# USCbiostats/fmcmc

Hardware: AMD Instinct MI355X
Metric: MH samples/sec (chains x iters / s), 1024 chains, 5-param linreg n=10k (higher is better)
Workload: dtype f64

## Files before the change

### fmcmc_amd/csrc/mh_spec.hpp

```cpp
#pragma once

namespace {

constexpr int SPEC_NT = 768;
constexpr int SPEC_NCW = 8;

__device__ __forceinline__ unsigned lds_ld_u32(const unsigned* p) {
  unsigned v;
  asm volatile("ds_read_b32 %0, %1\n\ts_waitcnt lgkmcnt(0)" : "=v"(v) : "v"((unsigned)(size_t)p) : "memory");
  return v;
}

__device__ __forceinline__ void lds_st_u32(unsigned* p, unsigned v) {
  asm volatile("ds_write_b32 %0, %1" : : "v"((unsigned)(size_t)p), "v"(v) : "memory");
}

__device__ __forceinline__ double lds_ld_f64(const double* p) {
  double v;
  asm volatile("ds_read_b64 %0, %1\n\ts_waitcnt lgkmcnt(0)" : "=v"(v) : "v"((unsigned)(size_t)p) : "memory");
  return v;
}



constexpr int SPEC_ALD = PIPE_KMAX + 1;
constexpr int SPEC_ADS = 7 * PIPE_KMAX + 2 * PIPE_KMAX * SPEC_ALD;

template <int KIND, class SYNC>
__device__ __forceinline__ void spec_owner_adaptive(const SweepArgs& A, int myc, int cl, double* s_th1, const double* s_par,
                                                    SYNC& sync, double* ad) {
  const int lane = threadIdx.x & 63;
  const int k = A.k, kz = A.kz, nsteps = (int)A.nsteps, burnin = (int)A.burnin, thin = (int)A.thin;
  constexpr int LD = SPEC_ALD;
  double* th0 = ad;
  double* th1 = th0 + PIPE_KMAX;
  double* vz = th1 + PIPE_KMAX;
  double* vv = vz + PIPE_KMAX;
  double* vmp = vv + PIPE_KMAX;
  double* vmt = vmp + PIPE_KMAX;
  double* vrs = vmt + PIPE_KMAX;
  double* SigA = vrs + PIPE_KMAX;
  double* SigB = SigA + PIPE_KMAX * LD;
  __shared__ int s_which[4][PIPE_KMAX];
  int kf = 0;
  for (int j = 0; j < k; j++)
    if (!A.fixed[j]) { if (lane == 0) s_which[myc][kf] = j; kf++; }
  const int* which = s_which[myc];
  const double* s_mu = s_par, *s_lb = s_par + 2 * PIPE_KMAX, *s_ub = s_par + 3 * PIPE_KMAX;
  double f0 = 0.0;
  long long abs_iter = 0;
  int nacc = 0, status = A.win_cont ? A.status[cl] : FMCMC_CHAIN_OK, thin_ctr = A.thin_ctr0, have_mean = 0, nerr = 0;
  const int ioff = (int)A.step_off;
  unsigned int bitword = 0;
  double* const Scur = SigA;
  if (lane < k) { double t = A.theta0[(long long)cl * k + lane]; th0[lane] = t; th1[lane] = t; }
  for (int e = lane; e < kf * LD; e += 64) {
    const int a = e / LD, b = e % LD;
    SigA[e] = A.fresh ? ((a == b) ? 1.0 * A.eps : 0.0) : ((b < kf && (b <= a || KIND == FMCMC_KERNEL_ADAPT)) ? A.Sigma[((long long)cl * kf + a) * kf + b] : 0.0);
    SigB[e] = 0.0;
  }
  if (!A.fresh) {
    abs_iter = A.abs_iter[cl];
    if (A.nerrors) nerr = A.nerrors[cl];
    if (KIND == FMCMC_KERNEL_ADAPT) {
      have_mean = A.have_mean[cl];
      if (lane < kf) vmp[lane] = A.mean_prev[(long long)cl * kf + lane];
    }
  }
  wave_sync_lds();
  const int jl = (lane < k) ? lane : 0;
  char* const s_base = reinterpret_cast<char*>(A.samples) + ((long long)cl * k) * A.ldS * 8;
  char* const d_base = A.draws ? reinterpret_cast<char*>(A.draws) + ((long long)cl * k) * A.ldS * 8 : nullptr;
  char* const l_base = A.logpost ? reinterpret_cast<char*>(A.logpost) + (long long)cl * A.ldS * 8 : nullptr;
  const unsigned int lane_off = (unsigned int)((long long)jl * A.ldS * 8);
  unsigned int srow8 = 0;
  const char* const z_base = reinterpret_cast<const char*>(A.fed_z) + ((long long)cl * nsteps) * kz * 8;
  const unsigned int z_lane = (unsigned int)((lane < kz ? lane : 0)) * 8u;
  const double* const lu_row = A.fed_logu + (long long)cl * nsteps;
  auto ld_z = [&](int row) -> double {
    return *reinterpret_cast<const double*>(z_base + (z_lane + (unsigned int)row * (unsigned int)(kz * 8)));
  };
  double z_nx = (lane < kz && nsteps >= 2) ? ld_z(1) : 0.0;
  double lu_nx = (nsteps >= 2) ? lu_row[1] : 0.0;
  bool ram_gate = false;
  auto flush_bits = [&](int i) {
    if (A.accept_bits && lane == 0) {
      unsigned int* w = A.accept_bits + ((long long)cl * A.bits_stride + ((i - 1) >> 5));
      *w = (A.win_cont && i <= 32) ? (*w | bitword) : bitword;
    }
    bitword = 0;
  };

  for (int v = 1; v <= nsteps; v++) {
    const double tot = sync.total(v, []() {});
    const double f1 = finish_logpost(A, th1, tot);
    bool keep_row = false, st_row = false;
    double st_th0 = 0.0, st_dr = 0.0;
    if (v == 1) {
      f0 = f1;
      if (lane < kf) vrs[lane] = (A.win_cont && A.win_sum) ? A.win_sum[(long long)cl * kf + lane] : th0[which[lane]];
      keep_row = true;
    } else if (status == FMCMC_CHAIN_OK) {
      const int i = v;
      if (KIND == FMCMC_KERNEL_RAM) {
        if (ram_gate) {
          double a_n = fmh_exp(f1 - f0);
          if (fmh_isnan(a_n)) a_n = 0.0;
          else if (a_n > 1.0) a_n = 1.0;
          double eta = (double)kf * fmh_exp(A.ram_neg_exp * fmh_log((double)(i + ioff)));
          if (eta > 1.0) eta = 1.0;
          const double zl = (lane < kf) ? vz[lane] : 0.0;
          const double Pj1 = lane_scan_row16(zl * zl);
          const double Pj = dpp_d<0x111>(Pj1);
          const double nrm2 = readlane_d(Pj1, kf - 1);
          double cp = (eta * (a_n - A.arate)) / nrm2;
          if (cp != 0.0 && fmh_isfinite(cp)) {
            double dl, kl;
            const bool okl = ram_coef(cp, Pj, Pj1, zl, dl, kl);
            if (__any(lane < kf && !okl)) {
              nerr += 1;
            } else {
              double* row = Scur + ((lane < kf) ? lane : 0) * LD;
              const double* grow = SigB + ((lane < kf) ? lane : 0) * LD;
              for (int j = 0; j < kf; j++) {
                const double dj = readlane_d(dl, j), kj = readlane_d(kl, j);
                const double sij = row[j];
                const double nw = fmh_fma(grow[j], kj, sij * dj);
                if (lane >= j && lane < kf) row[j] = nw;
              }
              wave_sync_lds();
            }
          }
        }
        abs_iter += 1;
      }
      if (fmh_isnan(f1)) status = FMCMC_CHAIN_NAN_LOGPOST;
      const double ratio = f1 - f0;
      if (status == FMCMC_CHAIN_OK && fmh_isnan(ratio)) status = FMCMC_CHAIN_NAN_RATIO;
      if (status != FMCMC_CHAIN_OK) {
        if (lane == 0) { A.status[cl] = status; A.status_step[cl] = i + ioff; }
        if (lane < k) A.status_theta[(long long)cl * k + lane] = th1[lane];
        flush_bits(i);
      } else {
        const double lu = lu_nx;
        lu_nx = lu_row[v < nsteps ? v : nsteps - 1];
        keep_row = true;
        if (i > burnin) {
          thin_ctr += 1;
        }
        const bool acc = lu < ratio;
        const double dr = (lane < k) ? th1[lane] : 0.0;
        if (acc) {
          if (lane < k) th0[lane] = dr;
          f0 = f1;
          nacc += 1;
          bitword |= (1u << ((i - 1) & 31));
        }
        wave_sync_lds();
        if (i > burnin && thin_ctr == thin) {
          thin_ctr = 0;
          st_row = true;
          st_th0 = (lane < k) ? th0[lane] : 0.0;
          st_dr = dr;
        }
        if (KIND == FMCMC_KERNEL_ADAPT && lane < kf) vrs[lane] = vrs[lane] + th0[which[lane]];
        if (((i - 1) & 31) == 31 || i == nsteps) flush_bits(i);
      }
    }
    if (v == 1 && keep_row && 1 > burnin) {
      thin_ctr += 1;
      if (thin_ctr == thin) {
        thin_ctr = 0;
        if (lane < k) {
          *reinterpret_cast<double*>(s_base + (lane_off + srow8)) = th0[lane];
          if (d_base) *reinterpret_cast<double*>(d_base + (lane_off + srow8)) = th1[lane];
        }
        if (l_base && lane == 0) *reinterpret_cast<double*>(l_base + srow8) = f1;
        srow8 += 8;
      }
    }
    if (v < nsteps) {
      if (status == FMCMC_CHAIN_OK) {
        const int i = v + 1;
        wave_sync_lds();
        if (lane < kz) vz[lane] = z_nx;
        z_nx = (lane < kz) ? ld_z(v + 1 < nsteps ? v + 1 : nsteps - 1) : 0.0;
        wave_sync_lds();
        if (KIND == FMCMC_KERNEL_ADAPT) {
          if (A.until > (double)abs_iter && abs_iter > A.warmup && i + ioff > 2) {
            const double t = (double)(abs_iter - 1);
            double x = 0, mp = 0, mt = 0;
            if (lane < kf) {
              x = th0[which[lane]];
              mp = have_mean ? vmp[lane] : (vrs[lane] / (double)(i + ioff - 1));
              mt = (mp * t + x) / (t + 1);
              vv[lane] = x; vmp[lane] = mp; vmt[lane] = mt;
            }
            wave_sync_lds();
            if (lane < kf) {
              const double c1 = (t - 1) / t, c2 = 1.0 / t;
              int b = 0;
              for (; b + 4 <= kf; b += 4) {
                double pb[4], tb[4], xb[4], sb[4];
#pragma unroll
                for (int u = 0; u < 4; u++) { pb[u] = vmp[b + u]; tb[u] = vmt[b + u]; xb[u] = vv[b + u]; sb[u] = SigA[lane * LD + b + u]; }
#pragma unroll
                for (int u = 0; u < 4; u++) {
                  const double ik = (b + u == lane) ? 1.0 * A.eps : 0.0;
                  const double inner = t * (mp * pb[u]) - (t + 1) * (mt * tb[u]) + x * xb[u] + 1e-5 * ik;
                  SigA[lane * LD + b + u] = c1 * sb[u] + c2 * inner;
                }
              }
              for (; b < kf; b++) {
                double ik = (b == lane) ? 1.0 * A.eps : 0.0;
                double inner = t * (mp * vmp[b]) - (t + 1) * (mt * vmt[b]) + x * vv[b] + 1e-5 * ik;
                SigA[lane * LD + b] = c1 * SigA[lane * LD + b] + c2 * inner;
              }
            }
            wave_sync_lds();
            if (lane < kf) vmp[lane] = mt;
            have_mean = 1;
          }
          abs_iter += 1;
          bool notpd = false;
          for (int j = 0; j < kf; j++) {
            double sacc = 0.0;
            if (lane >= j && lane < kf) {
              sacc = SigA[lane * LD + j];
              int b = 0;
              for (; b + 4 <= j; b += 4) {
                double lb4[4], wb4[4];
#pragma unroll
                for (int u = 0; u < 4; u++) { lb4[u] = SigB[lane * LD + b + u]; wb4[u] = SigB[(b + u) * LD + j]; }
#pragma unroll
                for (int u = 0; u < 4; u++) sacc = fmh_fma(-lb4[u], wb4[u], sacc);
              }
              for (; b < j; b++) sacc = fmh_fma(-SigB[lane * LD + b], SigB[b * LD + j], sacc);
            }
            const double d = readlane_d(sacc, j);
            if (!(d > 0.0) || !fmh_isfinite(d)) { notpd = true; break; }
            if (lane == j) { SigB[j * LD + j] = 1.0; vv[j] = d; }
            else if (lane > j && lane < kf) { SigB[lane * LD + j] = sacc / d; SigB[j * LD + lane] = sacc; }
            wave_sync_lds();
          }
          if (notpd) {
            status = FMCMC_CHAIN_NOT_PD;
            if (lane == 0) { A.status[cl] = status; A.status_step[cl] = i + ioff; }
            if (lane < k) A.status_theta[(long long)cl * k + lane] = th1[lane];
            if (((v - 1) & 31) != 31) flush_bits(v);
          } else {
            if (lane < k) th1[lane] = th0[lane];
            if (lane < kf) vz[lane] = fmh_sqrt(vv[lane]) * vz[lane];
            wave_sync_lds();
            if (lane < kf) {
              double sacc = 0.0;
              for (int b = 0; b < kf; b += 4) {
                double lb4[4], zb4[4];
#pragma unroll
                for (int u = 0; u < 4; u++) { const int bb = (b + u < kf) ? b + u : kf - 1; lb4[u] = SigB[lane * LD + bb]; zb4[u] = vz[bb]; }
#pragma unroll
                for (int u = 0; u < 4; u++) { const double nx = fmh_fma(lb4[u], zb4[u], sacc); sacc = (b + u <= lane) ? nx : sacc; }
              }
              const int j = which[lane];
              th1[j] = reflect1(th0[j] + (s_mu[j] + sacc), s_lb[j], s_ub[j]);
            }
          }
        } else {
          if (lane < kf) {
            double sacc = 0.0;
            for (int b = lane; b >= 0; b--) {
              SigB[lane * LD + b] = sacc;
              sacc = fmh_fma(Scur[lane * LD + b], vz[b], sacc);
            }
            const int j = which[lane];
            th1[j] = th0[j] + sacc;
          }
          ram_gate = (A.until > (double)abs_iter && abs_iter > A.warmup && ((v + 1 + ioff) % A.freq) == 0);
        }
        wave_sync_lds();
        if (lane < k) s_th1[myc * PIPE_KMAX + lane] = th1[lane];
      }
      sync.publish(v + 1);
    } else {
      sync.final();
    }
    if (st_row) {
      if (lane < k) {
        *reinterpret_cast<double*>(s_base + (lane_off + srow8)) = st_th0;
        if (d_base) *reinterpret_cast<double*>(d_base + (lane_off + srow8)) = st_dr;
      }
      if (l_base && lane == 0) *reinterpret_cast<double*>(l_base + srow8) = f1;
      srow8 += 8;
    }
  }
  wave_sync_lds();
  if (lane < k) A.theta0[(long long)cl * k + lane] = th0[lane];
  if (lane == 0) {
    A.f0[cl] = f0;
    A.accept_count[cl] = nacc;
    if (status == FMCMC_CHAIN_OK) { A.status[cl] = FMCMC_CHAIN_OK; A.status_step[cl] = 0; }
    A.abs_iter[cl] = abs_iter;
    if (A.nerrors) A.nerrors[cl] = nerr;
    if (KIND == FMCMC_KERNEL_ADAPT) A.have_mean[cl] = have_mean;
  }
  if (KIND == FMCMC_KERNEL_ADAPT && A.win_sum && lane < kf) A.win_sum[(long long)cl * kf + lane] = vrs[lane];
  const double* Sfin = (KIND == FMCMC_KERNEL_RAM) ? Scur : SigA;
  for (int e = lane; e < kf * kf; e += 64) {
    const int a = e / kf, b = e % kf;
    A.Sigma[((long long)cl * kf + a) * kf + b] = Sfin[a * LD + b];
  }
  if (KIND == FMCMC_KERNEL_ADAPT && lane < kf) A.mean_prev[(long long)cl * kf + lane] = vmp[lane];
}

constexpr int SPEC_KA = 8;

struct SpecSync {
  static constexpr bool PREP_EARLY = false;
  unsigned* s_ready; unsigned* s_done; const double* s_tr; int myc;
  template <class F> __device__ __forceinline__ double total(int v, F&&) const {
    const int lane = threadIdx.x & 63;
    while (lds_ld_u32(&s_done[myc]) < 8u * (unsigned)v) __builtin_amdgcn_s_sleep(1);
    const double* src = s_tr + myc * (8 * PIPE_TRS) + lane;
    const double v0 = src[0 * PIPE_TRS], v1 = src[1 * PIPE_TRS], v2 = src[2 * PIPE_TRS], v3 = src[3 * PIPE_TRS];
    const double v4 = src[4 * PIPE_TRS], v5 = src[5 * PIPE_TRS], v6 = src[6 * PIPE_TRS], v7 = src[7 * PIPE_TRS];
    return wave_xor_sum(((v0 + v1) + (v2 + v3)) + ((v4 + v5) + (v6 + v7)));
  }
  __device__ __forceinline__ void publish(int vn) const {
    asm volatile("s_waitcnt lgkmcnt(0)" ::: "memory");
    if ((threadIdx.x & 63) == 0) __hip_atomic_store(&s_ready[myc], (unsigned)vn, __ATOMIC_RELAXED, __HIP_MEMORY_SCOPE_WORKGROUP);
  }
  __device__ __forceinline__ void final() const {}
};
constexpr unsigned SPEC_FINAL = 0xFFFFFFFFu;
struct SpecSyncB {
  static constexpr bool PREP_EARLY = false;
  unsigned* s_ready; unsigned* s_done; const double* s_tr; int myc;
  mutable unsigned nreq = 1u;
  __device__ __forceinline__ double served() const {
    const int lane = threadIdx.x & 63;
    while (lds_ld_u32(&s_done[myc]) < 8u * nreq) __builtin_amdgcn_s_sleep(1);
    const double* src = s_tr + myc * (8 * PIPE_TRS) + lane;
    const double v0 = src[0 * PIPE_TRS], v1 = src[1 * PIPE_TRS], v2 = src[2 * PIPE_TRS], v3 = src[3 * PIPE_TRS];
    const double v4 = src[4 * PIPE_TRS], v5 = src[5 * PIPE_TRS], v6 = src[6 * PIPE_TRS], v7 = src[7 * PIPE_TRS];
    return wave_xor_sum(((v0 + v1) + (v2 + v3)) + ((v4 + v5) + (v6 + v7)));
  }
  __device__ __forceinline__ void ask() const {
    nreq += 1u;
    asm volatile("s_waitcnt lgkmcnt(0)" ::: "memory");
    if ((threadIdx.x & 63) == 0) __hip_atomic_store(&s_ready[myc], nreq, __ATOMIC_RELAXED, __HIP_MEMORY_SCOPE_WORKGROUP);
  }
  template <class F> __device__ __forceinline__ double total(int, F&&) const { return served(); }
  template <class W> __device__ __forceinline__ bool second(bool need, W&& republish, double& tot2) const {
    if (!need) return false;
    republish();
    ask();
    tot2 = served();
    return true;
  }
  __device__ __forceinline__ void second_idle() const {}
  __device__ __forceinline__ void publish(int) const { ask(); }
  __device__ __forceinline__ void final() const {
    if ((threadIdx.x & 63) == 0) __hip_atomic_store(&s_ready[myc], SPEC_FINAL, __ATOMIC_RELAXED, __HIP_MEMORY_SCOPE_WORKGROUP);
  }
};
constexpr int SPEC_FREQMAX = 8;
template <int KIND, int KX, class SYNC, bool BND = false, int FAM = FMCMC_FAM_GAUSSIAN_LINREG, bool RING = false>
__device__ __forceinline__ void spec_owner_adaptive_reg(const SweepArgs& A, int myc, int cl, double* s_th1, SYNC& sync,
                                                        double* ring = nullptr ) {
  static_assert(!BND || KIND == FMCMC_KERNEL_RAM, "BND is the bounded kernel_ram");
  constexpr bool LG = FAM == FMCMC_FAM_LOGISTIC;
  constexpr int KA = KX > 0 ? KX : SPEC_KA;
  const int lane = threadIdx.x & 63;
  const int k = KX > 0 ? KX : A.k, kz = KX > 0 ? KX : A.kz, kf = (KX > 0 || LG) ? k : kz;
  const int nsteps = (int)A.nsteps, burnin = (int)A.burnin, thin = (int)A.thin;
  const bool rl = lane < k;
  const int jl = rl ? lane : 0;
  const bool fl = lane < kf;
  int pj = jl, sig_lane = k - 1;
  if constexpr (KX == 0 && !LG) {
    int nfree = 0, nfix = 0, mine = 0;
    for (int j = 0; j < k; j++) {
      const bool fx = A.fixed[j] != 0;
      const int pos = fx ? (kf + nfix) : nfree;
      if (pos == lane) mine = j;
      if (j == k - 1) sig_lane = pos;
      nfree += fx ? 0 : 1; nfix += fx ? 1 : 0;
    }
    pj = rl ? mine : 0;
  }
  const double mu_l = A.mu[pj], lb_l = A.lb[pj], ub_l = A.ub[pj];
  double Srow[KA], Lrow[KA];
  double Wrow[KIND == FMCMC_KERNEL_ADAPT ? KA : 1];
  double (&Grow)[KA] = Lrow;
#pragma unroll
  for (int b = 0; b < (KIND == FMCMC_KERNEL_ADAPT ? KA : 1); b++) Wrow[b] = 0.0;
#pragma unroll
  for (int b = 0; b < KA; b++) {
    Lrow[b] = 0.0;
    Srow[b] = (fl && b < kf) ? (A.fresh ? ((b == lane) ? 1.0 * A.eps : 0.0)
                                        : ((b <= lane || KIND == FMCMC_KERNEL_ADAPT) ? A.Sigma[((long long)cl * kf + lane) * kf + b] : 0.0)) : 0.0;
  }
  double th0 = rl ? A.theta0[(long long)cl * k + pj] : 0.0, th1 = th0;
  double f0 = 0.0, mean_prev = 0.0, run_sum = 0.0, zcur = 0.0;
  double Dl = 0.0;
  long long abs_iter = 0;
  int nacc = 0, status = A.win_cont ? A.status[cl] : FMCMC_CHAIN_OK, thin_ctr = A.thin_ctr0, have_mean = 0, nerr = 0;
  const int ioff = (int)A.step_off;
  unsigned int bitword = 0;
  if (!A.fresh) {
    abs_iter = A.abs_iter[cl];
    if (A.nerrors) nerr = A.nerrors[cl];
    if (KIND == FMCMC_KERNEL_ADAPT) {
      have_mean = A.have_mean[cl];
      if (fl) mean_prev = A.mean_prev[(long long)cl * kf + lane];
    }
  }
  char* const s_base = reinterpret_cast<char*>(A.samples) + ((long long)cl * k) * A.ldS * 8;
  char* const d_base = A.draws ? reinterpret_cast<char*>(A.draws) + ((long long)cl * k) * A.ldS * 8 : nullptr;
  char* const l_base = A.logpost ? reinterpret_cast<char*>(A.logpost) + (long long)cl * A.ldS * 8 : nullptr;
  const unsigned int lane_off = (unsigned int)((long long)pj * A.ldS * 8);
  unsigned int srow8 = 0;
  const char* const z_base = reinterpret_cast<const char*>(A.fed_z) + ((long long)cl * nsteps) * kz * 8;
  const unsigned int z_lane = (unsigned int)(fl ? lane : 0) * 8u;
  const double* const lu_row = A.fed_logu + (long long)cl * nsteps;
  const double dn = uniform_d((double)A.n);
  auto ld_z = [&](int row) -> double {
    return *reinterpret_cast<const double*>(z_base + (z_lane + (unsigned int)row * (unsigned int)(kz * 8)));
  };
  double z_nx = (fl && nsteps >= 2) ? ld_z(1) : 0.0;
  double lu_nx = (nsteps >= 2) ? lu_row[1] : 0.0;
  bool ram_gate = false;
  auto flush_bits = [&](int i) {
    if (A.accept_bits && lane == 0) {
      unsigned int* w = A.accept_bits + ((long long)cl * A.bits_stride + ((i - 1) >> 5));
      *w = (A.win_cont && i <= 32) ? (*w | bitword) : bitword;
    }
    bitword = 0;
  };
  auto logpost_of = [&](double tot, double sigma) -> double {
    double f;
    if (sigma < 0.0 || fmh_isnan(sigma)) f = fmh_nan();
    else if (sigma == 0.0) f = -fmh_inf();
    else {
      double t1 = fmh_log(sigma) + FMH_K(FMH_LN_SQRT_2PI);
      double q = (0.5 * tot) / (sigma * sigma);
      f = -(dn * t1) - q;
    }
    if (A.guard && !fmh_isfinite(f)) f = -fmh_inf();
    return f;
  };

  double pre_nt1 = 0.0, pre_ss = 1.0, pre_rs = 1.0, pre_eta = 0.0, pre_Pj = 0.0, pre_Pj1 = 0.0, pre_nrm2 = 1.0;
  double pre_c1 = 0.0, pre_c2 = 0.0;
  double pre_lin = 0.0, pre_pri = 0.0;
  const int nbl = A.intercept + A.p;
  const double hs_l = (LG && lane < nbl && A.lg_hs) ? A.lg_hs[lane] : 0.0;
  bool pre_ok = false;
  auto prepare = [&](int i) {
    if (KIND == FMCMC_KERNEL_ADAPT) {
      const double t = uniform_d((double)(abs_iter - 1));
      pre_c1 = (t - 1) / t;
      pre_c2 = 1.0 / t;
    }
    if constexpr (LG) {
      double lin = 0.0, ss = 0.0;
      for (int j = 0; j < nbl; j++) {
        const double bj = readlane_d(th1, j);
        lin = fmh_fma(bj, readlane_d(hs_l, j), lin);
        ss = fmh_fma(bj, bj, ss);
      }
      pre_lin = lin;
      pre_pri = (A.prior_div != 0.0) ? ss / A.prior_div : 0.0;
      if (KIND == FMCMC_KERNEL_RAM && i >= 2) {
        double eta = (double)kf * fmh_exp(A.ram_neg_exp * fmh_log((double)(i + ioff)));
        if (eta > 1.0) eta = 1.0;
        pre_eta = eta;
        pre_Pj1 = lane_scan_row16(zcur * zcur);
        pre_Pj = dpp_d<0x111>(pre_Pj1);
        pre_nrm2 = readlane_d(pre_Pj1, kf - 1);
      }
      return;
    }
    const double sigma = readlane_d(th1, sig_lane);
    const unsigned sg_hi = (unsigned)(fmh_d2u(sigma) >> 32);
    const bool sg_fast = (sg_hi - 0x00100000u) < 0x7fe00000u;
    const double sg = sg_fast ? sigma : 1.0;
    pre_nt1 = dn * (fmh_log(sg) + FMH_K(FMH_LN_SQRT_2PI));
    pre_ss = sg * sg;
    pre_ok = sg_fast && mfr_div_safe(pre_ss);
    pre_rs = div_recip(pre_ok ? pre_ss : 1.0);
    if (KIND == FMCMC_KERNEL_RAM && i >= 2) {
      double eta = (double)kf * fmh_exp(A.ram_neg_exp * fmh_log((double)(i + ioff)));
      if (eta > 1.0) eta = 1.0;
      pre_eta = eta;
      pre_Pj1 = lane_scan_row16(zcur * zcur);
      pre_Pj = dpp_d<0x111>(pre_Pj1);
      pre_nrm2 = readlane_d(pre_Pj1, kf - 1);
    }
  };
  if (!SYNC::PREP_EARLY) prepare(1);
#ifdef SPEC_STAMP
  unsigned long long stt[8] = {0, 0, 0, 0, 0, 0, 0, 0}, stp = clk();
#define SPEC_ST(i) do { const unsigned long long t_ = clk(); stt[i] += t_ - stp; stp = t_; } while (0)
#else
#define SPEC_ST(i) do { } while (0)
#endif

  for (int v = 1; v <= nsteps; v++) {
    const double tot = sync.total(v, [&]() { prepare(v); });
    SPEC_ST(0);
    const double h = 0.5 * tot;
    double f1;
    if constexpr (LG) {
      f1 = pre_lin - tot;
      if (A.prior_div != 0.0) f1 = f1 - pre_pri;
      if (A.guard && !fmh_isfinite(f1)) f1 = -fmh_inf();
    } else if (pre_ok && mfr_div_safe(h)) f1 = -pre_nt1 - div_finish(h, pre_ss, pre_rs);
    else f1 = logpost_of(tot, readlane_d(th1, sig_lane));
    bool st_row = false;
    double st_th0 = 0.0;
    double st_dr = th1;
    SPEC_ST(1);
    if (v == 1) {
      f0 = f1;
      run_sum = (A.win_cont && A.win_sum && fl) ? A.win_sum[(long long)cl * kf + lane] : th0;
      if (1 > burnin) { thin_ctr += 1; if (thin_ctr == thin) { thin_ctr = 0; st_row = true; st_th0 = th0; } }
      if constexpr (BND) sync.second_idle();
    } else if (status != FMCMC_CHAIN_OK) {
      if constexpr (BND) sync.second_idle();
    } else {
      const int i = v;
      if (KIND == FMCMC_KERNEL_RAM) {
        if (ram_gate) {
          double a_n = fmh_exp(f1 - f0);
          if (fmh_isnan(a_n)) a_n = 0.0;
          else if (a_n > 1.0) a_n = 1.0;
          const double eta = pre_eta, Pj1 = pre_Pj1, Pj = pre_Pj, nrm2 = pre_nrm2;
          const double cp = (eta * (a_n - A.arate)) / nrm2;
          if (cp != 0.0 && fmh_isfinite(cp)) {
            double dl, kl;
            const bool okl = ram_coef(cp, Pj, Pj1, zcur, dl, kl);
            if (__any(fl && !okl)) {
              nerr += 1;
            } else {
              static_for<KA>([&](auto j_) {
                constexpr int j = decltype(j_)::value;
                if (j < kf) {
                  const double dj = row_bcast<j>(dl), kj = row_bcast<j>(kl);
                  Srow[j] = fmh_fma(Grow[j], kj, Srow[j] * dj);
                }
              });
            }
          }
        }
        abs_iter += 1;
        if constexpr (BND) {
          const double th1r = fl ? reflect1(th1, lb_l, ub_l) : th1;
          const bool moved = __any(fl && !(th1r == th1));
          th1 = th1r;
          st_dr = th1r;
          double tot2 = 0.0;
          const bool again = sync.second(moved, [&]() { if (rl) s_th1[myc * PIPE_KMAX + pj] = th1; }, tot2);
          if (again && moved) {
            if constexpr (LG) {
              double lin = 0.0, ss = 0.0;
              for (int j = 0; j < nbl; j++) {
                const double bj = readlane_d(th1, j);
                lin = fmh_fma(bj, readlane_d(hs_l, j), lin);
                ss = fmh_fma(bj, bj, ss);
              }
              f1 = lin - tot2;
              if (A.prior_div != 0.0) f1 = f1 - ss / A.prior_div;
              if (A.guard && !fmh_isfinite(f1)) f1 = -fmh_inf();
            } else {
              f1 = logpost_of(tot2, readlane_d(th1, sig_lane));
            }
          }
        }
      }
      if (fmh_isnan(f1)) status = FMCMC_CHAIN_NAN_LOGPOST;
      const double ratio = f1 - f0;
      if (status == FMCMC_CHAIN_OK && fmh_isnan(ratio)) status = FMCMC_CHAIN_NAN_RATIO;
      if (status != FMCMC_CHAIN_OK) {
        if (lane == 0) { A.status[cl] = status; A.status_step[cl] = i + ioff; }
        if (rl) A.status_theta[(long long)cl * k + pj] = th1;
        flush_bits(i);
      } else {
        const double lu = lu_nx;
        lu_nx = lu_row[v < nsteps ? v : nsteps - 1];
        if (lu < ratio) {
          th0 = th1;
          f0 = f1;
          nacc += 1;
          bitword |= (1u << ((i - 1) & 31));
        }
        if (i > burnin) { thin_ctr += 1; if (thin_ctr == thin) { thin_ctr = 0; st_row = true; st_th0 = th0; } }
        if (KIND == FMCMC_KERNEL_ADAPT) run_sum = run_sum + th0;
        if (((i - 1) & 31) == 31 || i == nsteps) flush_bits(i);
      }
    }
    SPEC_ST(2);
    const int afreq = (KIND == FMCMC_KERNEL_ADAPT && RING) ? A.freq : 1;
    if (KIND == FMCMC_KERNEL_ADAPT && afreq > 1 && ring && fl) ring[(v & (SPEC_FREQMAX - 1)) * PIPE_KMAX + lane] = th0;
    if (v < nsteps) {
      if (status == FMCMC_CHAIN_OK) {
        const int i = v + 1;
        zcur = z_nx;
        z_nx = fl ? ld_z(v + 1 < nsteps ? v + 1 : nsteps - 1) : 0.0;
        bool sig_dirty = (afreq == 1) || v == 1;
        if (KIND == FMCMC_KERNEL_ADAPT) {
          if (A.until > (double)abs_iter && abs_iter > A.warmup && i + ioff > 2 && (afreq == 1 || ((i + ioff) % afreq) == 0)) {
            if (afreq > 1 && i - afreq < 1) {
              status = FMCMC_CHAIN_BAD_WINDOW;
            } else {
              for (int jr = 0; jr < afreq; jr++) {
                const double t = (double)(abs_iter - afreq + jr);
                const double x = (afreq == 1) ? th0 : (fl ? ring[((i - afreq + jr) & (SPEC_FREQMAX - 1)) * PIPE_KMAX + lane] : 0.0);
                const double mp = have_mean ? mean_prev : (run_sum / (double)(i + ioff - 1));
                const double mt = (mp * t + x) / (t + 1);
                const double c1 = (afreq == 1) ? pre_c1 : (t - 1) / t, c2 = (afreq == 1) ? pre_c2 : 1.0 / t;
                static_for<KA>([&](auto b_) {
                  constexpr int b = decltype(b_)::value;
                  if (b < kf) {
                    const double mpb = row_bcast<b>(mp), mtb = row_bcast<b>(mt), xb = row_bcast<b>(x);
                    const double ik = (b == lane) ? 1.0 * A.eps : 0.0;
                    const double inner = t * (mp * mpb) - (t + 1) * (mt * mtb) + x * xb + 1e-5 * ik;
                    Srow[b] = c1 * Srow[b] + c2 * inner;
                  }
                });
                mean_prev = mt;
                have_mean = 1;
              }
              sig_dirty = true;
            }
          }
          abs_iter += 1;
          SPEC_ST(3);
          bool notpd = false;
          if (!RING || (status == FMCMC_CHAIN_OK && sig_dirty)) {
          Dl = 0.0;
          static_for<KA>([&](auto j_) {
            constexpr int j = decltype(j_)::value;
            if (j < kf && (KX > 0 || !notpd)) {
              double sacc = Srow[j];
              static_for<j>([&](auto b_) {
                constexpr int b = decltype(b_)::value;
                sacc = fmac_row_bcast<j, true>(sacc, Wrow[KIND == FMCMC_KERNEL_ADAPT ? b : 0], Lrow[b]);
              });
              const double d = readlane_d(sacc, j);
              const bool badp = !(d > 0.0) || !fmh_isfinite(d);
              if (KX > 0) notpd = notpd || badp;
              if (KX <= 0 && badp) {
                notpd = true;
              } else {
                const double qj = sacc / d;
                Lrow[j] = (lane == j) ? 1.0 : ((lane > j) ? qj : Lrow[j]);
                Wrow[KIND == FMCMC_KERNEL_ADAPT ? j : 0] = sacc;
                Dl = (lane == j) ? d : Dl;
              }
            }
          });
          }
          SPEC_ST(4);
          if (notpd || (RING && status != FMCMC_CHAIN_OK)) {
            if (notpd) status = FMCMC_CHAIN_NOT_PD;
            if (lane == 0) { A.status[cl] = status; A.status_step[cl] = i + ioff; }
            if (rl) A.status_theta[(long long)cl * k + pj] = th1;
            if (((v - 1) & 31) != 31) flush_bits(v);
          } else {
            const double ul = fmh_sqrt(Dl) * zcur;
            double sacc = 0.0;
            static_for<KA>([&](auto b_) {
              constexpr int b = decltype(b_)::value;
              if (b < kf) sacc = fmac_row_bcast<b>(sacc, ul, Lrow[b]);
            });
            th1 = (KX != 0 || LG || fl) ? reflect1(th0 + (mu_l + sacc), lb_l, ub_l) : th0;
          }
        } else {
          double sacc = 0.0;
          static_for<KA>([&](auto r_) {
            constexpr int b = KA - 1 - decltype(r_)::value;
            if (b < kf) { Grow[b] = sacc; sacc = fmac_row_bcast<b>(sacc, zcur, Srow[b]); }
          });
          th1 = (KX != 0 || LG || fl) ? th0 + sacc : th0;
          ram_gate = (A.until > (double)abs_iter && abs_iter > A.warmup && ((v + 1 + ioff) % A.freq) == 0);
        }
        if (rl) s_th1[myc * PIPE_KMAX + pj] = th1;
      }
      sync.publish(v + 1);
    } else {
      sync.final();
    }
    SPEC_ST(5);
    if (st_row) {
      if (rl) {
        *reinterpret_cast<double*>(s_base + (lane_off + srow8)) = st_th0;
        if (d_base) *reinterpret_cast<double*>(d_base + (lane_off + srow8)) = st_dr;
      }
      if (l_base && lane == 0) *reinterpret_cast<double*>(l_base + srow8) = f1;
      srow8 += 8;
    }
    SPEC_ST(6);
    if (!SYNC::PREP_EARLY && v < nsteps) prepare(v + 1);
    SPEC_ST(7);
  }
#ifdef SPEC_STAMP
  __builtin_amdgcn_s_waitcnt(0);
  if (lane < 16 && A.draws) A.draws[(long long)cl * 16 + lane] = (lane < 8) ? (double)stt[lane & 7] : (double)nsteps;
#endif
#undef SPEC_ST
  if (rl) A.theta0[(long long)cl * k + pj] = th0;
  if (lane == 0) {
    A.f0[cl] = f0;
    A.accept_count[cl] = nacc;
    if (status == FMCMC_CHAIN_OK) { A.status[cl] = FMCMC_CHAIN_OK; A.status_step[cl] = 0; }
    A.abs_iter[cl] = abs_iter;
    if (A.nerrors) A.nerrors[cl] = nerr;
    if (KIND == FMCMC_KERNEL_ADAPT) A.have_mean[cl] = have_mean;
  }
#pragma unroll
  for (int b = 0; b < KA; b++)
    if (fl && b < kf) A.Sigma[((long long)cl * kf + lane) * kf + b] = (b <= lane || KIND == FMCMC_KERNEL_ADAPT) ? Srow[b] : 0.0;
  if (KIND == FMCMC_KERNEL_ADAPT && fl) A.mean_prev[(long long)cl * kf + lane] = mean_prev;
  if (KIND == FMCMC_KERNEL_ADAPT && A.win_sum && fl) A.win_sum[(long long)cl * kf + lane] = run_sum;
}

template <int KIND, class SYNC>
__device__ __forceinline__ void mfma_owner_mirror(const SweepArgs& A, int myc, int cl, double* s_th1, SYNC& sync) {
  const int lane = threadIdx.x & 63;
  const int k = A.k, kz = A.kz;
  const int nsteps = (int)A.nsteps, burnin = (int)A.burnin, thin = (int)A.thin;
  const bool rl = lane < k;
  const int jl = rl ? lane : 0;
  const double lb_l = A.lb[jl], ub_l = A.ub[jl];
  double th0 = rl ? A.theta0[(long long)cl * k + lane] : 0.0, th1 = th0;
  double mmu = rl ? (A.fresh ? A.mu[jl] : A.mirror_mu[(long long)cl * k + jl]) : 0.0;
  double msc = rl ? (A.fresh ? A.scale[jl] : A.mirror_scale[(long long)cl * k + jl]) : 0.0;
  double f0 = 0.0, obs_arate = fmh_nan(), th_prev = 0.0;
  long long abs_iter = 0, nzero = 0;
  if (!A.fresh) { abs_iter = A.abs_iter[cl]; obs_arate = A.obs_arate[(long long)cl * k + jl]; }
  int nacc = 0, status = FMCMC_CHAIN_OK, thin_ctr = 0;
  unsigned int bitword = 0;
  char* const s_base = reinterpret_cast<char*>(A.samples) + ((long long)cl * k) * A.ldS * 8;
  char* const d_base = A.draws ? reinterpret_cast<char*>(A.draws) + ((long long)cl * k) * A.ldS * 8 : nullptr;
  char* const l_base = A.logpost ? reinterpret_cast<char*>(A.logpost) + (long long)cl * A.ldS * 8 : nullptr;
  const unsigned int lane_off = (unsigned int)((long long)jl * A.ldS * 8);
  unsigned int srow8 = 0;
  const char* const z_base = reinterpret_cast<const char*>(A.fed_z) + ((long long)cl * nsteps) * kz * 8;
  const unsigned int z_lane = (unsigned int)(jl) * 8u;
  const double* const lu_row = A.fed_logu + (long long)cl * nsteps;
  const double dn = uniform_d((double)A.n);
  auto ld_z = [&](int row) -> double { return *reinterpret_cast<const double*>(z_base + (z_lane + (unsigned int)row * (unsigned int)(kz * 8))); };
  double z_nx = (rl && nsteps >= 2) ? ld_z(1) : 0.0;
  double lu_nx = (nsteps >= 2) ? lu_row[1] : 0.0;
  auto flush_bits = [&](int i) {
    if (A.accept_bits && lane == 0) A.accept_bits[(long long)cl * ((nsteps + 31) >> 5) + ((i - 1) >> 5)] = bitword;
    bitword = 0;
  };
  auto logpost_of = [&](double tot, double sigma) -> double {
    double f;
    if (sigma < 0.0 || fmh_isnan(sigma)) f = fmh_nan();
    else if (sigma == 0.0) f = -fmh_inf();
    else {
      double t1 = fmh_log(sigma) + FMH_K(FMH_LN_SQRT_2PI);
      double q = (0.5 * tot) / (sigma * sigma);
      f = -(dn * t1) - q;
    }
    if (A.guard && !fmh_isfinite(f)) f = -fmh_inf();
    return f;
  };
  double pre_nt1 = 0.0, pre_ss = 1.0, pre_rs = 1.0, pre_den = 1.0, pre_rd = 1.0;
  bool pre_ok = false;
  auto prepare = [&]() {
    const double sigma = readlane_d(th1, k - 1);
    const unsigned sg_hi = (unsigned)(fmh_d2u(sigma) >> 32);
    const bool sg_fast = (sg_hi - 0x00100000u) < 0x7fe00000u;
    const double sg = sg_fast ? sigma : 1.0;
    pre_nt1 = dn * (fmh_log(sg) + FMH_K(FMH_LN_SQRT_2PI));
    pre_ss = sg * sg;
    pre_ok = sg_fast && mfr_div_safe(pre_ss);
    pre_rs = div_recip(pre_ok ? pre_ss : 1.0);
    pre_den = (double)abs_iter + 1;
    pre_rd = div_recip(pre_den);
  };
  auto over_den = [&](double num) -> double {
    if (__all(!rl || mfr_div_safe(num))) return div_finish(num, pre_den, pre_rd);
    return num / pre_den;
  };
  if (!SYNC::PREP_EARLY) prepare();
  for (int v = 1; v <= nsteps; v++) {
    const double tot = sync.total(v, [&]() { prepare(); });
    const double hq = 0.5 * tot;
    const double f1 = (pre_ok && mfr_div_safe(hq)) ? (-pre_nt1 - div_finish(hq, pre_ss, pre_rs)) : logpost_of(tot, readlane_d(th1, k - 1));
    bool st_row = false;
    double st_th0 = 0.0;
    const double st_dr = th1;
    if (v == 1) {
      f0 = f1;
      if (1 > burnin) { thin_ctr += 1; if (thin_ctr == thin) { thin_ctr = 0; st_row = true; st_th0 = th0; } }
    } else if (status == FMCMC_CHAIN_OK) {
      const int i = v;
      if (fmh_isnan(f1)) status = FMCMC_CHAIN_NAN_LOGPOST;
      const double ratio = f1 - f0;
      if (status == FMCMC_CHAIN_OK && fmh_isnan(ratio)) status = FMCMC_CHAIN_NAN_RATIO;
      if (status != FMCMC_CHAIN_OK) {
        if (lane == 0) { A.status[cl] = status; A.status_step[cl] = i; }
        if (rl) A.status_theta[(long long)cl * k + lane] = th1;
        flush_bits(i);
      } else {
        const double lu = lu_nx;
        lu_nx = lu_row[v < nsteps ? v : nsteps - 1];
        bool moved = false;
        th_prev = th0;
        if (lu < ratio) {
          const double d = th1 - th0;
          moved = __any(rl && (d * d != 0.0));
          th0 = th1;
          f0 = f1;
          nacc += 1;
          bitword |= (1u << ((i - 1) & 31));
        }
        if (!moved) nzero += 1;
        if (i > burnin) { thin_ctr += 1; if (thin_ctr == thin) { thin_ctr = 0; st_row = true; st_th0 = th0; } }
        if (((i - 1) & 31) == 31 || i == nsteps) flush_bits(i);
      }
    }
    if (v < nsteps) {
      if (status == FMCMC_CHAIN_OK) {
        const int i = v + 1;
        const double z = z_nx;
        z_nx = rl ? ld_z(v + 1 < nsteps ? v + 1 : nsteps - 1) : 0.0;
        if (abs_iter >= 1 && abs_iter <= A.warmup) mmu = over_den(mmu * (double)abs_iter + th0);
        if (abs_iter == A.nadapt) {
          obs_arate = 1.0 - (double)nzero / (double)(i - 2);
          const double num = fmh_tan_0_halfpi(1.5707963267948966 * obs_arate);
          const double den = fmh_tan_0_halfpi(1.5707963267948966 * A.arate);
          msc = msc * num / den;
        } else if (abs_iter > A.nadapt && abs_iter <= A.warmup) {
          obs_arate = (i < 3) ? fmh_nan() : over_den(obs_arate * (double)abs_iter + ((th0 != th_prev) ? 1.0 : 0.0));
        }
        double t;
        if (KIND == FMCMC_KERNEL_NMIRROR) {
          t = (2.0 * mmu - th0) + msc * z;
        } else {
          const double sqrt3 = fmh_sqrt(3.0);
          const double c = 2.0 * mmu - th0;
          const double lo = c - sqrt3 * msc, hi = c + sqrt3 * msc;
          t = lo + (hi - lo) * z;
        }
        th1 = reflect1(t, lb_l, ub_l);
        abs_iter += 1;
        if (rl) s_th1[myc * PIPE_KMAX + lane] = th1;
      }
      sync.publish(v + 1);
    } else {
      sync.final();
    }
    if (st_row) {
      if (rl) {
        *reinterpret_cast<double*>(s_base + (lane_off + srow8)) = st_th0;
        if (d_base) *reinterpret_cast<double*>(d_base + (lane_off + srow8)) = st_dr;
      }
      if (l_base && lane == 0) *reinterpret_cast<double*>(l_base + srow8) = f1;
      srow8 += 8;
    }
    if (!SYNC::PREP_EARLY && v < nsteps) prepare();
  }
  if (rl) {
    A.theta0[(long long)cl * k + lane] = th0;
    A.mirror_mu[(long long)cl * k + lane] = mmu;
    A.mirror_scale[(long long)cl * k + lane] = msc;
    A.obs_arate[(long long)cl * k + lane] = obs_arate;
  }
  if (lane == 0) {
    A.f0[cl] = f0;
    A.accept_count[cl] = nacc;
    if (status == FMCMC_CHAIN_OK) { A.status[cl] = FMCMC_CHAIN_OK; A.status_step[cl] = 0; }
    A.abs_iter[cl] = abs_iter;
  }
}

template <int P, int OPT, bool BNDC = false>
__device__ __forceinline__ void spec_compute(const SweepArgs& A, const double* s_y, const double* s_th1, unsigned* s_ready, unsigned* s_done,
                                             double* s_tr, int ncw, int nsteps, int ic, bool dbg, int wave, int tid, int lane,
                                             const unsigned* = nullptr) {
    double xr[OPT][P > 0 ? P : 1];
    double wlast = 1.0, wprev = 1.0;
#pragma unroll
    for (int s = 0; s < OPT; s++) {
      const long long i = (long long)tid + (long long)NT * s;
      const bool valid = i < A.n;
#pragma unroll
      for (int j = 0; j < P; j++) xr[s][j] = valid ? A.X[(long long)j * A.n + i] : 0.0;
      if (s == OPT - 1) wlast = valid ? 1.0 : 0.0;
      if (s == OPT - 2) wprev = valid ? 1.0 : 0.0;
    }
    const int tr_slot = (tid & 7) * PIPE_TRS + (tid >> 3);
    const double2* yp = reinterpret_cast<const double2*>(s_y) + tid;
    unsigned long long tw = 0, te = 0;
    unsigned srv0 = 0u, srv1 = 0u, srv2 = 0u, srv3 = 0u;
    unsigned live = BNDC ? ((1u << ncw) - 1u) : 0u;
    for (int v = 1; BNDC ? (live != 0u) : (v <= nsteps); v++) {
      for (int c = 0; c < ncw; c++) {
        unsigned long long t_a = dbg ? clk() : 0;
        if constexpr (BNDC) {
          if (!((live >> c) & 1u)) continue;
          const unsigned mine = c == 0 ? srv0 : (c == 1 ? srv1 : (c == 2 ? srv2 : srv3));
          unsigned w;
          while ((w = (unsigned)__builtin_amdgcn_readfirstlane((int)lds_ld_u32(&s_ready[c]))) <= mine) __builtin_amdgcn_s_sleep(1);
          if (w == SPEC_FINAL) { live &= ~(1u << c); continue; }
          srv0 += (c == 0) ? 1u : 0u; srv1 += (c == 1) ? 1u : 0u; srv2 += (c == 2) ? 1u : 0u; srv3 += (c == 3) ? 1u : 0u;
        } else {
          while (lds_ld_u32(&s_ready[c]) < (unsigned)v) __builtin_amdgcn_s_sleep(1);
        }
        unsigned long long t_b = dbg ? clk() : 0;
        const double* t0 = s_th1 + c * PIPE_KMAX;
        const double m00 = ic ? t0[0] : 0.0;
        double b0[P > 0 ? P : 1];
#pragma unroll
        for (int j = 0; j < P; j++) b0[j] = t0[ic + j];
        double a0 = 0.0;
        constexpr int YD = 3;
        double2 yq[YD];
#pragma unroll
        for (int d = 0; d < YD; d++) yq[d] = yp[(d < OPT / 2 ? d : OPT / 2 - 1) * NT];
#pragma unroll
        for (int s2 = 0; s2 < OPT / 2; s2++) {
          const double2 yy = yq[s2 % YD];
          if (s2 + YD < OPT / 2) yq[s2 % YD] = yp[(s2 + YD) * NT];
#pragma unroll
          for (int h = 0; h < 2; h++) {
            const int s = 2 * s2 + h;
            const double yv = h ? yy.y : yy.x;
            double m0 = m00;
#pragma unroll
            for (int j = 0; j < P; j++) m0 = fmh_fma(xr[s][j], b0[j], m0);
            const double r0 = yv - m0;
            if (s == OPT - 1) a0 = fmh_fma(r0 * wlast, r0, a0);
            else if (s == OPT - 2) a0 = fmh_fma(r0 * wprev, r0, a0);
            else a0 = fmh_fma(r0, r0, a0);
          }
        }
        s_tr[c * (8 * PIPE_TRS) + tr_slot] = a0;
        asm volatile("s_waitcnt lgkmcnt(0)" ::: "memory");
        if (lane == 0) __hip_atomic_fetch_add(&s_done[c], 1u, __ATOMIC_RELAXED, __HIP_MEMORY_SCOPE_WORKGROUP);
        if (dbg) { unsigned long long t_c = clk(); tw += t_b - t_a; te += t_c - t_b; }
      }
    }
    if (dbg && lane == 0 && A.draws) {
      double* d = A.draws + ((long long)blockIdx.x * 12 + wave) * 4;
      d[0] = (double)tw; d[1] = (double)te; d[2] = 0.0; d[3] = (double)nsteps;
    }
}

template <int P, int OPT, bool BNDC = false>
__device__ __forceinline__ void spec_compute_logit(const SweepArgs& A, const double* s_tab, const double* s_th1, unsigned* s_ready, unsigned* s_done,
                                                   double* s_tr, int ncw, int nsteps, int ic, int wave, int tid, int lane) {
    double xr[OPT][P > 0 ? P : 1];
    double wlast = 1.0, wprev = 1.0;
#pragma unroll
    for (int s = 0; s < OPT; s++) {
      const long long i = (long long)tid + (long long)NT * s;
      const bool valid = i < A.n;
#pragma unroll
      for (int j = 0; j < P; j++) xr[s][j] = valid ? A.X[(long long)j * A.n + i] : 0.0;
      if (s == OPT - 1) wlast = valid ? 1.0 : 0.0;
      if (s == OPT - 2) wprev = valid ? 1.0 : 0.0;
    }
    const int tr_slot = (tid & 7) * PIPE_TRS + (tid >> 3);
    unsigned srv0 = 0u, srv1 = 0u, srv2 = 0u, srv3 = 0u;
    unsigned live = BNDC ? ((1u << ncw) - 1u) : 0u;
    for (int v = 1; BNDC ? (live != 0u) : (v <= nsteps); v++) {
      for (int c = 0; c < ncw; c++) {
        if constexpr (BNDC) {
          if (!((live >> c) & 1u)) continue;
          const unsigned mine = c == 0 ? srv0 : (c == 1 ? srv1 : (c == 2 ? srv2 : srv3));
          unsigned w;
          while ((w = (unsigned)__builtin_amdgcn_readfirstlane((int)lds_ld_u32(&s_ready[c]))) <= mine) __builtin_amdgcn_s_sleep(1);
          if (w == SPEC_FINAL) { live &= ~(1u << c); continue; }
          srv0 += (c == 0) ? 1u : 0u; srv1 += (c == 1) ? 1u : 0u; srv2 += (c == 2) ? 1u : 0u; srv3 += (c == 3) ? 1u : 0u;
        } else {
          while (lds_ld_u32(&s_ready[c]) < (unsigned)v) __builtin_amdgcn_s_sleep(1);
        }
        const double* t0 = s_th1 + c * PIPE_KMAX;
        const double m00 = ic ? t0[0] * FMH_LG_SCALE : 0.0;
        double b0[P > 0 ? P : 1];
#pragma unroll
        for (int j = 0; j < P; j++) b0[j] = t0[ic + j] * FMH_LG_SCALE;
        double a0 = 0.0;
        constexpr int G = 4;
#pragma unroll
        for (int s0 = 0; s0 < OPT; s0 += G) {
          constexpr int GG = G;
          double us[GG], gv[GG];
#pragma unroll
          for (int u = 0; u < GG; u++) {
            double es = m00;
            if (s0 + u < OPT) {
#pragma unroll
// ... 301 lines not shown
```

Measured before the change: 496.9 million.

## Cut register pressure in spec MH loop via scalarized state and cold kernarg reloads

Rare-path fields (accept_bits, status, guard, win_sum, step_off) are now reloaded from the kernarg segment through an opaque pointer instead of being kept live in registers. Loop-invariant status values are made wave-uniform with readfirstlane, and the adaptation gate is precomputed once as an iteration range [gate_lo, gate_hi). Error-handling branches are marked unlikely and merged into a shared stop_chain helper, and the st_th0 temporary is removed. The goal is to lower VGPR/SGPR pressure and per-iteration scalar work in the hot loop. The risks are subtle semantic drift, for example in the gate computation when until is not an integer, and NaN detection becoming wave-level via __any.

```diff
diff --git a/fmcmc_amd/csrc/mh_spec.hpp b/fmcmc_amd/csrc/mh_spec.hpp
--- a/fmcmc_amd/csrc/mh_spec.hpp
+++ b/fmcmc_amd/csrc/mh_spec.hpp
@@ -314,12 +314,21 @@
 
 constexpr int SPEC_KA = 8;
 
+typedef const SweepArgs __attribute__((address_space(4))) SweepArgsK;
+__device__ __forceinline__ SweepArgsK* sweep_args_cold() {
+  SweepArgsK* p = (SweepArgsK*)__builtin_amdgcn_kernarg_segment_ptr();
+#if defined(__HIP_DEVICE_COMPILE__)
+  asm volatile("" : "+s"(p));
+#endif
+  return p;
+}
+
 struct SpecSync {
   static constexpr bool PREP_EARLY = false;
   unsigned* s_ready; unsigned* s_done; const double* s_tr; int myc;
   template <class F> __device__ __forceinline__ double total(int v, F&&) const {
     const int lane = threadIdx.x & 63;
-    while (lds_ld_u32(&s_done[myc]) < 8u * (unsigned)v) __builtin_amdgcn_s_sleep(1);
+    while ((unsigned)__builtin_amdgcn_readfirstlane((int)lds_ld_u32(&s_done[myc])) < 8u * (unsigned)v) __builtin_amdgcn_s_sleep(1);
     const double* src = s_tr + myc * (8 * PIPE_TRS) + lane;
     const double v0 = src[0 * PIPE_TRS], v1 = src[1 * PIPE_TRS], v2 = src[2 * PIPE_TRS], v3 = src[3 * PIPE_TRS];
     const double v4 = src[4 * PIPE_TRS], v5 = src[5 * PIPE_TRS], v6 = src[6 * PIPE_TRS], v7 = src[7 * PIPE_TRS];
@@ -338,7 +347,7 @@
   mutable unsigned nreq = 1u;
   __device__ __forceinline__ double served() const {
     const int lane = threadIdx.x & 63;
-    while (lds_ld_u32(&s_done[myc]) < 8u * nreq) __builtin_amdgcn_s_sleep(1);
+    while ((unsigned)__builtin_amdgcn_readfirstlane((int)lds_ld_u32(&s_done[myc])) < 8u * nreq) __builtin_amdgcn_s_sleep(1);
     const double* src = s_tr + myc * (8 * PIPE_TRS) + lane;
     const double v0 = src[0 * PIPE_TRS], v1 = src[1 * PIPE_TRS], v2 = src[2 * PIPE_TRS], v3 = src[3 * PIPE_TRS];
     const double v4 = src[4 * PIPE_TRS], v5 = src[5 * PIPE_TRS], v6 = src[6 * PIPE_TRS], v7 = src[7 * PIPE_TRS];
@@ -404,16 +413,30 @@
   double f0 = 0.0, mean_prev = 0.0, run_sum = 0.0, zcur = 0.0;
   double Dl = 0.0;
   long long abs_iter = 0;
-  int nacc = 0, status = A.win_cont ? A.status[cl] : FMCMC_CHAIN_OK, thin_ctr = A.thin_ctr0, have_mean = 0, nerr = 0;
+  int nacc = 0, status = A.win_cont ? __builtin_amdgcn_readfirstlane(A.status[cl]) : FMCMC_CHAIN_OK, thin_ctr = A.thin_ctr0, have_mean = 0, nerr = 0;
   const int ioff = (int)A.step_off;
   unsigned int bitword = 0;
   if (!A.fresh) {
     abs_iter = A.abs_iter[cl];
     if (A.nerrors) nerr = A.nerrors[cl];
     if (KIND == FMCMC_KERNEL_ADAPT) {
-      have_mean = A.have_mean[cl];
+      have_mean = __builtin_amdgcn_readfirstlane(A.have_mean[cl]);
       if (fl) mean_prev = A.mean_prev[(long long)cl * kf + lane];
     }
+  }
+  int gate_lo, gate_hi;
+  {
+    const long long abs0 = abs_iter;
+    long long lo = (long long)A.warmup - abs0 + 1;
+    if (KIND == FMCMC_KERNEL_ADAPT && lo < 1 - (long long)ioff) lo = 1 - (long long)ioff;
+    gate_lo = (int)(lo < 0 ? 0 : (lo > nsteps ? nsteps : lo));
+    const double until = A.until;
+    long long hi = 0;
+    if (until >= 9007199254740992.0) hi = (long long)nsteps + 1;
+    else if (until > 0.0) hi = (long long)__builtin_ceil(until) - abs0 + 1;
+    gate_hi = (int)(hi < 0 ? 0 : (hi > (long long)nsteps + 1 ? (long long)nsteps + 1 : hi));
+    gate_lo = __builtin_amdgcn_readfirstlane(gate_lo);
+    gate_hi = __builtin_amdgcn_readfirstlane(gate_hi);
   }
   char* const s_base = reinterpret_cast<char*>(A.samples) + ((long long)cl * k) * A.ldS * 8;
   char* const d_base = A.draws ? reinterpret_cast<char*>(A.draws) + ((long long)cl * k) * A.ldS * 8 : nullptr;
@@ -431,11 +454,19 @@
   double lu_nx = (nsteps >= 2) ? lu_row[1] : 0.0;
   bool ram_gate = false;
   auto flush_bits = [&](int i) {
-    if (A.accept_bits && lane == 0) {
-      unsigned int* w = A.accept_bits + ((long long)cl * A.bits_stride + ((i - 1) >> 5));
-      *w = (A.win_cont && i <= 32) ? (*w | bitword) : bitword;
+    SweepArgsK* const C = sweep_args_cold();
+    unsigned int* const bits = C->accept_bits;
+    if (bits && lane == 0) {
+      unsigned int* w = bits + ((long long)cl * C->bits_stride + ((i - 1) >> 5));
+      *w = (C->win_cont && i <= 32) ? (*w | bitword) : bitword;
     }
     bitword = 0;
+  };
+  auto stop_chain = [&](int i, int flush_i) {
+    SweepArgsK* const C = sweep_args_cold();
+    if (lane == 0) { C->status[cl] = status; C->status_step[cl] = i + (int)C->step_off; }
+    if (lane < k) C->status_theta[(long long)cl * k + pj] = th1;
+    if (flush_i > 0) flush_bits(flush_i);
   };
   auto logpost_of = [&](double tot, double sigma) -> double {
     double f;
@@ -446,7 +477,7 @@
       double q = (0.5 * tot) / (sigma * sigma);
       f = -(dn * t1) - q;
     }
-    if (A.guard && !fmh_isfinite(f)) f = -fmh_inf();
+    if (sweep_args_cold()->guard && !fmh_isfinite(f)) f = -fmh_inf();
     return f;
   };
 
@@ -515,18 +546,19 @@
       f1 = pre_lin - tot;
       if (A.prior_div != 0.0) f1 = f1 - pre_pri;
       if (A.guard && !fmh_isfinite(f1)) f1 = -fmh_inf();
-    } else if (pre_ok && mfr_div_safe(h)) f1 = -pre_nt1 - div_finish(h, pre_ss, pre_rs);
+    } else if (__builtin_expect(pre_ok && __all(mfr_div_safe(h)), 1)) f1 = -pre_nt1 - div_finish(h, pre_ss, pre_rs);
     else f1 = logpost_of(tot, readlane_d(th1, sig_lane));
     bool st_row = false;
-    double st_th0 = 0.0;
     double st_dr = th1;
     SPEC_ST(1);
-    if (v == 1) {
+    if (__builtin_expect(v == 1, 0)) {
       f0 = f1;
-      run_sum = (A.win_cont && A.win_sum && fl) ? A.win_sum[(long long)cl * kf + lane] : th0;
-      if (1 > burnin) { thin_ctr += 1; if (thin_ctr == thin) { thin_ctr = 0; st_row = true; st_th0 = th0; } }
+      SweepArgsK* const C = sweep_args_cold();
+      double* const wsum = C->win_sum;
+      run_sum = (C->win_cont && wsum && fl) ? wsum[(long long)cl * kf + lane] : th0;
+      if (1 > burnin) { thin_ctr += 1; if (thin_ctr == thin) { thin_ctr = 0; st_row = true; } }
       if constexpr (BND) sync.second_idle();
-    } else if (status != FMCMC_CHAIN_OK) {
+    } else if (__builtin_expect(status != FMCMC_CHAIN_OK, 0)) {
       if constexpr (BND) sync.second_idle();
     } else {
       const int i = v;
@@ -578,13 +610,10 @@
           }
         }
       }
-      if (fmh_isnan(f1)) status = FMCMC_CHAIN_NAN_LOGPOST;
       const double ratio = f1 - f0;
-      if (status == FMCMC_CHAIN_OK && fmh_isnan(ratio)) status = FMCMC_CHAIN_NAN_RATIO;
-      if (status != FMCMC_CHAIN_OK) {
-        if (lane == 0) { A.status[cl] = status; A.status_step[cl] = i + ioff; }
-        if (rl) A.status_theta[(long long)cl * k + pj] = th1;
-        flush_bits(i);
+      if (__builtin_expect(__any(fmh_isnan(f1) || fmh_isnan(ratio)), 0)) {
+        status = __any(fmh_isnan(f1)) ? FMCMC_CHAIN_NAN_LOGPOST : FMCMC_CHAIN_NAN_RATIO;
+        stop_chain(i, i);
       } else {
         const double lu = lu_nx;
         lu_nx = lu_row[v < nsteps ? v : nsteps - 1];
@@ -594,9 +623,9 @@
           nacc += 1;
           bitword |= (1u << ((i - 1) & 31));
         }
-        if (i > burnin) { thin_ctr += 1; if (thin_ctr == thin) { thin_ctr = 0; st_row = true; st_th0 = th0; } }
+        if (i > burnin) { thin_ctr += 1; if (thin_ctr == thin) { thin_ctr = 0; st_row = true; } }
         if (KIND == FMCMC_KERNEL_ADAPT) run_sum = run_sum + th0;
-        if (((i - 1) & 31) == 31 || i == nsteps) flush_bits(i);
+        if (__builtin_expect(((i - 1) & 31) == 31 || i == nsteps, 0)) flush_bits(i);
       }
     }
     SPEC_ST(2);
@@ -609,14 +638,16 @@
         z_nx = fl ? ld_z(v + 1 < nsteps ? v + 1 : nsteps - 1) : 0.0;
         bool sig_dirty = (afreq == 1) || v == 1;
         if (KIND == FMCMC_KERNEL_ADAPT) {
-          if (A.until > (double)abs_iter && abs_iter > A.warmup && i + ioff > 2 && (afreq == 1 || ((i + ioff) % afreq) == 0)) {
+          if (v > gate_lo && v < gate_hi && (afreq == 1 || ((i + ioff) % afreq) == 0)) {
             if (afreq > 1 && i - afreq < 1) {
               status = FMCMC_CHAIN_BAD_WINDOW;
             } else {
               for (int jr = 0; jr < afreq; jr++) {
                 const double t = (double)(abs_iter - afreq + jr);
                 const double x = (afreq == 1) ? th0 : (fl ? ring[((i - afreq + jr) & (SPEC_FREQMAX - 1)) * PIPE_KMAX + lane] : 0.0);
-                const double mp = have_mean ? mean_prev : (run_sum / (double)(i + ioff - 1));
+                double mp = mean_prev;
+                if constexpr (RING) mp = have_mean ? mean_prev : (run_sum / (double)(i + ioff - 1));
+                else if (__builtin_expect(!have_mean, 0)) mp = run_sum / (double)(i + (int)sweep_args_cold()->step_off - 1);
                 const double mt = (mp * t + x) / (t + 1);
                 const double c1 = (afreq == 1) ? pre_c1 : (t - 1) / t, c2 = (afreq == 1) ? pre_c2 : 1.0 / t;
                 static_for<KA>([&](auto b_) {
@@ -662,11 +693,9 @@
           });
           }
           SPEC_ST(4);
-          if (notpd || (RING && status != FMCMC_CHAIN_OK)) {
+          if (__builtin_expect(notpd || (RING && status != FMCMC_CHAIN_OK), 0)) {
             if (notpd) status = FMCMC_CHAIN_NOT_PD;
-            if (lane == 0) { A.status[cl] = status; A.status_step[cl] = i + ioff; }
-            if (rl) A.status_theta[(long long)cl * k + pj] = th1;
-            if (((v - 1) & 31) != 31) flush_bits(v);
+            stop_chain(i, (((v - 1) & 31) != 31) ? v : 0);
           } else {
             const double ul = fmh_sqrt(Dl) * zcur;
             double sacc = 0.0;
@@ -683,7 +712,7 @@
             if (b < kf) { Grow[b] = sacc; sacc = fmac_row_bcast<b>(sacc, zcur, Srow[b]); }
           });
           th1 = (KX != 0 || LG || fl) ? th0 + sacc : th0;
-          ram_gate = (A.until > (double)abs_iter && abs_iter > A.warmup && ((v + 1 + ioff) % A.freq) == 0);
+          ram_gate = (v > gate_lo && v < gate_hi && ((v + 1 + ioff) % A.freq) == 0);
         }
         if (rl) s_th1[myc * PIPE_KMAX + pj] = th1;
       }
@@ -694,7 +723,7 @@
     SPEC_ST(5);
     if (st_row) {
       if (rl) {
-        *reinterpret_cast<double*>(s_base + (lane_off + srow8)) = st_th0;
+        *reinterpret_cast<double*>(s_base + (lane_off + srow8)) = th0;
         if (d_base) *reinterpret_cast<double*>(d_base + (lane_off + srow8)) = st_dr;
       }
       if (l_base && lane == 0) *reinterpret_cast<double*>(l_base + srow8) = f1;
```

Result: no change. 496.8 million (-0.0%).
